# hku-mars/LiDAR_IMU_Init

Hardware: AMD Instinct MI355X
Metric: ICP+ESKF scans/sec @100k pts/scan (higher is better)
Workload: dtype f64; 1 GPU; stream100k: 100000 pts/scan (time-sorted) vs 1000000-pt local map, max_iteration 5, LIO mode (12-col H), static map, voxel-grid leaf 0.05; scans resident in HBM, 8 distinct scans cycled, the state reset to the scan's propagated state every step; map_points=1000000, params=harness/launch/ouster (reference-format yaml + launch), parallelism=points sharded x1, transport=none, rccl_ranks=0

## Files before the change

lidar_imu_init_amd/csrc/lii_capi_register.cpp:

```cpp
#include "lii_context.h"
#include <cstddef>

#include "lii_hostmath.h"

using namespace lii_impl;

namespace {


int next_knn_epoch(lii_handle h) {
  h->knn_epoch = h->knn_epoch >= 0x3FFFFFFE ? 1 : h->knn_epoch + 1;
  return h->knn_epoch;
}
void launch_knn(lii_handle h, const GridView& g, const RegistrationBuffers& rb, const PoseArg* pose, int forced, int epoch,
                hipEvent_t ev_start = nullptr, hipEvent_t ev_stop = nullptr) {
  lii::launch_knn(g, rb, pose, h->d_ctrl, forced, h->d_ctrl->search_pose, h->stream, epoch, ev_start, ev_stop);
}


int iterate(lii_handle h, const lii_state* st, bool search, bool imu_en, double* out91) {
  if (h->n_body <= 0) return fail(h, LII_ERR_STATE, "no down-sampled scan (call lii_downsample / lii_downsample_skip)");
  int rc = commit_map(h);
  if (rc != LII_OK) return rc;
  if (!search && !h->have_search) return fail(h, LII_ERR_STATE, "non-search iteration before any search");
  GridView g = grid_view(h);
  RegistrationBuffers rb = reg_buffers(h);
  const bool prof = h->prof.profiling;
  if (prof) HIPCHK(h, hipEventRecord(h->prof.ev[0], h->stream));
  {
    PoseArg* stage = reinterpret_cast<PoseArg*>(h->h_small + 20000);
    *stage = pose_of(*st);
    HIPCHK(h, hipMemcpyAsync(h->d_pose, stage, sizeof(PoseArg), hipMemcpyHostToDevice, h->stream));
  }
  if (search) h->unfinished_known = false;
  const int epoch = search ? next_knn_epoch(h) : 0;
  if (search) launch_knn(h, g, rb, h->d_pose, 1, epoch);
  if (prof) HIPCHK(h, hipEventRecord(h->prof.ev[3], h->stream));
  launch_fit_reduce(g, rb, h->d_pose, h->d_ctrl, search ? 1 : 0, imu_en ? 1 : 0, h->cfg.plane_threshold,
                    h->cfg.laser_point_cov_inv, h->stream, epoch);
  if (prof) HIPCHK(h, hipEventRecord(h->prof.ev[1], h->stream));
  launch_reduce91(rb, h->d_out91, h->d_ctrl, 1, h->stream, epoch);
  if (prof) HIPCHK(h, hipEventRecord(h->prof.ev[2], h->stream));
  if (search) h->have_search = true;
  if (h->net.comm) {
    ncclResult_t r = ncclAllReduce(h->d_out91, h->d_out91, kNormalEq, ncclDouble, ncclSum, h->net.comm, h->stream);
    if (r != ncclSuccess) return fail(h, LII_ERR_COMM, std::string("ncclAllReduce: ") + ncclGetErrorString(r));
  } else if (h->net.mailbox.dev_slots) {
    launch_mailbox_allreduce(h->d_out91, mailbox_view(h), h->stream);
  }
  HIPCHK(h, hipMemcpyAsync(h->h_small, h->d_out91, sizeof(double) * kNormalEq, hipMemcpyDeviceToHost, h->stream));
  HIPCHK(h, hipStreamSynchronize(h->stream));
  std::memcpy(out91, h->h_small, sizeof(double) * kNormalEq);
  if (h->net.mailbox.dev_slots && out91[kNormalEq - 1] != out91[kNormalEq - 1])
    return fail(h, LII_ERR_COMM, "mailbox exchange timed out (a rank of the job did not reach this pass)");
  if (prof) {
    float a = 0, b = 0;
    HIPCHK(h, hipEventElapsedTime(&a, h->prof.ev[0], h->prof.ev[1]));
    HIPCHK(h, hipEventElapsedTime(&b, h->prof.ev[1], h->prof.ev[2]));
    if (search) {
      float k = 0;
      HIPCHK(h, hipEventElapsedTime(&k, h->prof.ev[0], h->prof.ev[3]));
      h->prof.timings[0] += a; h->prof.timings[5] += 1; h->prof.timings[7] += k;
    } else { h->prof.timings[1] += a; h->prof.timings[6] += 1; }
    h->prof.timings[2] += b;
  }
  return LII_OK;
}

void fill_ctrl(lii_handle h, const lii_state* state, const lii_state* state_prop, const lii_iekf_opts* opts) {
  IekfCtrl* hc = h->h_ctrl;
  std::memcpy(hc->st, state, sizeof(lii_state));
  std::memcpy(hc->prop, state_prop, sizeof(hc->prop));
  hc->max_it = opts->max_iterations;
  hc->imu_en = opts->imu_en;
  hc->it = 0; hc->search_next = 1; hc->stop = 0; hc->rematch_num = 0; hc->converged = 0; hc->searches = 0;
  hc->effect_num = 0; hc->singular = 0;
  h->update_seq = h->update_seq == 0x7FFFFFFF ? 1 : h->update_seq + 1;
  hc->seq = h->update_seq;
  unsigned int plan = 0xFFFFFFFFu;
  if (h->knn_plan && !h->net.comm && opts->max_iterations <= 16) {
    plan = (h->knn_plan_force >= 0 ? ((unsigned int)h->knn_plan_force | 0xFFFF0000u) : h->plan_next) | 0x00010001u;
  }
  hc->plan_mask = plan;
  h->plan_cur = plan;
}

int update_on_device(lii_handle h, lii_state* state, const lii_state* state_prop, const lii_iekf_opts* opts,
                     lii_iekf_report* report) {
  static_assert(sizeof(lii_state) == sizeof(double) * kStateDoubles, "lii_state layout");
  if (h->n_body <= 0) return fail(h, LII_ERR_STATE, "no down-sampled scan (call lii_downsample / lii_downsample_skip)");
  const auto t_map0 = std::chrono::steady_clock::now();
  int rc = commit_map(h);
  if (rc != LII_OK) return rc;
  if (h->diag) h->prof.host_map_us[0] += std::chrono::duration<double, std::micro>(std::chrono::steady_clock::now() - t_map0).count();
  hipStream_t s = h->stream;
  if (!h->map_stream && h->net.n_ranks <= 1) HIPCHK(h, h->map_stream.create(hipStreamNonBlocking));
  if (!h->ctrl_preloaded) {
    if (h->staging_busy) HIPCHK(h, hipStreamSynchronize(s));
    fill_ctrl(h, state, state_prop, opts);
    HIPCHK(h, hipMemcpyAsync(h->d_ctrl, h->h_ctrl, sizeof(IekfCtrl), hipMemcpyHostToDevice, s));
  }
  h->ctrl_preloaded = false;
  h->h_res->singular = 0;
  h->h_res->it = -1;
  if (h->lm.in_job) {
    rc = local_map_enqueue(h, h->d_ctrl->st + 9, nullptr, h->prof.kp_active);
    if (rc != LII_OK) return rc;
  }
  GridView g = grid_view(h);
  RegistrationBuffers rb = reg_buffers(h);
  const PoseArg* pose = reinterpret_cast<const PoseArg*>(h->d_ctrl);
  const bool prof = h->prof.profiling && h->prof.prof_mode != 3;
  if (prof) harvest_knn_events(h);
  const double* ne = h->net.comm ? h->d_out91 + 128 : h->d_out91;
  unsigned int plan = h->plan_cur;
  const unsigned int plan0 = plan;
  auto enqueue_pass = [&](int it) -> int {
    const bool knn = it >= 16 || ((plan >> it) & 1u);
    const int epoch = knn ? next_knn_epoch(h) : 0;
    if (knn) {
      if (h->prof.kp_active) { const int r = kp_mark(h, LII_KP_KNN, it); if (r != LII_OK) return r; }
      if (prof && it < 16) launch_knn(h, g, rb, pose, -1, epoch, h->prof.ev_it[2 * it], h->prof.ev_it[2 * it + 1]);
      else launch_knn(h, g, rb, pose, -1, epoch);
    }
    if (h->prof.kp_active) { const int r = kp_mark(h, LII_KP_FIT, it); if (r != LII_OK) return r; }
    if (knn && h->wide_listed && !h->net.comm && h->net.n_ranks <= 1) launch_complete_listed(g, rb, h->d_ctrl, -1, s, epoch);
    launch_fit_reduce(g, rb, pose, h->d_ctrl, -1, opts->imu_en ? 1 : 0, h->cfg.plane_threshold, h->cfg.laser_point_cov_inv, s, epoch);
    if (h->prof.kp_active) { const int r = kp_mark(h, LII_KP_SOLVE, it); if (r != LII_OK) return r; }
    if (!h->net.comm) {
      launch_reduce_solve(rb, h->d_gran, h->d_ctrl, h->h_res, mailbox_view(h), s, epoch);
      return LII_OK;
    }
    launch_reduce91(rb, h->d_out91, h->d_ctrl, -1, s, epoch);
    ncclResult_t r = ncclAllReduce(h->d_out91, h->d_out91 + 128, kNormalEq, ncclDouble, ncclSum, h->net.comm, s);
    if (r != ncclSuccess) return fail(h, LII_ERR_COMM, std::string("ncclAllReduce: ") + ncclGetErrorString(r));
    launch_iekf_solve(h->d_ctrl, ne, h->h_res, s);
    return LII_OK;
  };
  const auto t_loop0 = std::chrono::steady_clock::now();
  for (int it = 0; it < opts->max_iterations; it++) {
    if (it < 16 && !((plan >> (16 + it)) & 1u)) break;
    rc = enqueue_pass(it);
    if (rc != LII_OK) return rc;
  }
  auto wait_result = [&](bool first) -> int {
    const int parked_word = first ? (h->update_seq | kLoopParked) : h->update_seq;
    if (h->poll_result && !h->net.comm) {
      volatile int* done = &h->h_res->done;
      unsigned int spins = 0;
      while (*done != h->update_seq && *done != parked_word) {
        if ((++spins & 0x3FFF) == 0) {
          const hipError_t q = hipStreamQuery(s);
          if (q == hipSuccess) break;
          if (q != hipErrorNotReady) return fail(h, LII_ERR_HIP, std::string("hipStreamQuery: ") + hipGetErrorString(q));
        }
        __builtin_ia32_pause();
      }
      std::atomic_thread_fence(std::memory_order_acquire);
      if (*done != h->update_seq && *done != parked_word) HIPCHK(h, hipStreamSynchronize(s));
    } else {
      HIPCHK(h, hipStreamSynchronize(s));
    }
    return LII_OK;
  };
  if (h->diag) h->prof.host_loop_enq_us = std::chrono::duration<double, std::micro>(std::chrono::steady_clock::now() - t_loop0).count();
  if (h->prof.kp_active) { rc = kp_mark(h, LII_KP_KINDS); if (rc != LII_OK) return rc; }
  h->map_enqueued_early = false;
  if (h->map_after_update && !h->net.comm && !h->prof.profiling) {
    const auto t_me0 = std::chrono::steady_clock::now();
    h->map_enqueued_early = map_update_early(h) == 1;
    g = grid_view(h);
    if (h->diag) h->prof.host_map_us[1] += std::chrono::duration<double, std::micro>(std::chrono::steady_clock::now() - t_me0).count();
  }
  if (h->pub.on) { rc = publish_enqueue(h, h->d_ctrl, nullptr, true); if (rc != LII_OK) return rc; }
  if (h->pre.want_dev && !h->net.comm && h->net.n_ranks <= 1 && h->prof.prof_mode != 3 && !h->map_async && h->poll_result) {
    lii::GateState* gst = h->pre.state;
    h->pre.seq = (h->pre.seq + 1) & 0x003FFFFFFFFFFFFFull;
    __atomic_store_n(&gst->word, (h->pre.seq << 2) | lii::kGateArmed, __ATOMIC_RELEASE);
    h->pre.scan_dev = h->pre.want_dev; h->pre.n = h->pre.want_n; h->pre.leaf = h->pre.want_leaf; h->pre.late = h->pre.want_late;
    h->pre.fuse = fuse_filter(h, h->pre.leaf);
    DeskewPlan dp = {};
    dp.in = static_cast<const float4*>(h->pre.scan_dev);
    dp.out = h->pre.late ? const_cast<float4*>(dp.in) : h->d_scan;
    dp.n = h->pre.n; dp.sorted = 1; dp.extent = nullptr; dp.bbox_rows = h->d_bbox_rows;
    dp.leaf = h->pre.leaf; dp.vh = h->pre.fuse ? &h->vh : nullptr;
    dp.ctrl_src = h->h_ctrl; dp.ctrl_dst = h->d_ctrl; dp.ctrl_bytes = (sizeof(IekfCtrl) + 15) / 16 * 16;
#ifdef LII_GAP_TRACE
    dp.gap = h->d_gran;
#endif
    lii::DeskewGate gate = {gst, h->pre.d_ring + size_t(h->pre.seq % lii::kGateRing) * lii::kGateLines * 8, h->pre.d_flag, h->pre.seq, h->pre.timeout_ticks, h->pre.late ? 1 : 0};
    launch_deskew_imu_gated(dp, gate, s);
    h->pre.armed = hipGetLastError() == hipSuccess;
    if (!h->pre.armed) __atomic_store_n(&gst->word, (h->pre.seq << 2) | lii::kGateCancel, __ATOMIC_RELEASE);
  }
  h->pre.want_dev = nullptr;
  if (h->wait_hook) {
    void (*hook)(void*) = h->wait_hook;
    h->wait_hook = nullptr;
    h->in_wait_hook = true;
    hook(h->wait_hook_arg);
    h->in_wait_hook = false;
  }
  rc = wait_result(true);
  if (rc != LII_OK) return rc;
  bool parked_once = false;
  for (int round = 0; h->h_res->done == (h->update_seq | kLoopParked); round++) {
    if (round > 2 * opts->max_iterations) return fail(h, LII_ERR_HIP, "device loop parked again and again");
    parked_once = true;
    const int from = h->h_res->parked_it;
    const bool search = h->h_res->parked_search != 0;
    h->plan_parked++;
    prearm_cancel(h);
    h->map_enqueued_early = false;
    g = grid_view(h);
    const int last = std::min(opts->max_iterations, std::max(h->plan_passes_prev, from + 1));
    unsigned int rplan = 0u;
    for (int q = from; q < last && q < 16; q++) rplan |= 1u << (16 + q);
    if (search && from < 16) rplan |= 1u << from;
    plan = rplan;
    h->h_res->done = 0;
    std::atomic_thread_fence(std::memory_order_release);
    launch_loop_resume(h->d_ctrl, rplan, s);
    for (int it = from; it < last; it++) {
      rc = enqueue_pass(it);
      if (rc != LII_OK) return rc;
    }
    if (h->prof.kp_active) { rc = kp_mark(h, LII_KP_KINDS); if (rc != LII_OK) return rc; }
    rc = wait_result(true);
    if (rc != LII_OK) return rc;
  }
  if (h->pub.on && parked_once) {
    if (h->pub.kp_idx >= 0) h->prof.kp_kind[size_t(h->pub.kp_idx)] = LII_KP_KINDS * 64;
    rc = publish_enqueue(h, h->d_ctrl, nullptr, false);
    if (rc != LII_OK) return rc;
  }
  h->unfinished_known = !h->net.comm;
  if (!h->net.comm && h->wide_enabled) {
    const bool wide = h->h_res->unfinished > lii::kFlagCap;
    if (wide == h->wide_prev && wide != h->wide_listed) { h->wide_listed = wide; h->wide_switches++; }
    h->wide_prev = wide;
    if (wide) h->wide_scans++;
  }
  h->staging_busy = false;
  h->scan_buf_idle = !h->pub.on;
  const IekfResult* hr = h->h_res;
  h->have_search = true;
#ifdef LII_SOLVE_TRACE
  {
    static int cnt = 0;
    if (++cnt % 100 == 0) {
      auto row = [&](const long long* t) {
        fprintf(stderr, " loads+sums %lld | A %lld | elimination %lld | solution %lld | state %lld | cov %lld ;", t[1] - t[0], t[2] - t[1], t[4] - t[3], t[8] - t[4],
                t[9] - t[8], t[10] - t[9]);
      };
      fprintf(stderr, "[solve trace, 10 ns ticks] stopping pass:");
      row(hr->ts);
      fprintf(stderr, "  pass 0:");
      row(hr->ts0);
      fprintf(stderr, "\n");
    }
  }
#endif
  if (h->prof.kp_active && h->prof.kp_n > 1 && hr->it > 0) {
    HIPCHK(h, hipEventSynchronize(h->prof.kp_ev[size_t(h->prof.kp_n - 1)]));
    for (int i = 0; i + 1 < h->prof.kp_n; i++) {
      int kind = h->prof.kp_kind[size_t(i)] / 64;
      const int it = h->prof.kp_kind[size_t(i)] % 64;
      if (kind >= LII_KP_KINDS) continue;
      const bool loop_kind = kind == LII_KP_KNN || kind == LII_KP_FIT || kind == LII_KP_SOLVE;
      if (loop_kind && (it >= hr->it || it >= 16)) continue;
      if (kind == LII_KP_KNN && !(hr->search_log[it] & 1)) continue;
      if (kind == LII_KP_FIT && (hr->search_log[it] & 1)) kind = LII_KP_FIT_SEARCH;
      float ms = 0;
      if (hipEventElapsedTime(&ms, h->prof.kp_ev[size_t(i)], h->prof.kp_ev[size_t(i + 1)]) != hipSuccess) continue;
      h->prof.kprof.ms[kind] += ms;
      h->prof.kprof.launches[kind] += 1;
    }
    h->prof.kprof.scans += 1;
  }
  if (hr->part_overflow) {
    h->h_res->part_overflow = 0;
    return fail(h, LII_ERR_CAPACITY, "voxel-partitioned job: this rank's share of the down-sampled cloud exceeds its bound (mean share + 25 % + 2048 points); use lii_comm_set_partition(h, 1)");
  }
  if (hr->singular == 3)
    return fail(h, LII_ERR_COMM, "mailbox exchange timed out (a rank of the job did not reach this pass); re-create the communicator");
  if (hr->singular == 4)
    return fail(h, LII_ERR_COMM, "the sums of a pass did not reach the solver within 2 s (a summing workgroup of the launch was not scheduled: is the device shared?)");
  if (hr->singular) return fail(h, LII_ERR_INVALID, "singular covariance / normal matrix in the device solve");
  if (hr->it < 0) return fail(h, LII_ERR_HIP, "device loop ended without a result");
  std::memcpy(state, hr->st, sizeof(lii_state));
  publish_finish(h);
  h->last_pivoted_passes = 0;
  for (int q = 0; q < 16 && q < hr->it; q++) h->last_pivoted_passes += (hr->search_log[q] >> 1) & 1;
  {
    unsigned int next = 0xFFFFFFFFu;
    for (int q = 0; q < 16 && q < hr->it; q++)
      if (!(hr->search_log[q] & 1)) next &= ~(1u << q);
    for (int q = std::max(hr->it, h->plan_passes_prev); q < 16; q++) next &= ~(1u << (16 + q));
    h->plan_passes_prev = hr->it;
    h->plan_next = next;
  }
  if (report) {
    report->iterations = hr->it;
    report->searches = hr->searches;
    report->effect_num = hr->effect_num;
    report->converged = hr->converged;
    std::memcpy(report->normal_eq, hr->ne, sizeof(double) * kNormalEq);
  }
  if (prof) {
    unsigned int due = 0u;
    for (int it = 0; it < opts->max_iterations && it < 16; it++) {
      if (it >= hr->it || !(hr->search_log[it] & 1) || !((plan0 >> it) & 1u)) continue;
      due |= 1u << it;
    }
    h->prof.ev_it_due = due;
  }
  return LII_OK;
}



int imu_prologue(lii_handle h, const lii_scan_job* job, const ImuFeed* feed, const lii_state* state, bool adopt, const float4* src_dev, int n_next,
                 bool sorted) {
  if (n_next <= 0) return fail(h, LII_ERR_STATE, "lii_scan_register_imu: no scan (lii_scan_upload / lii_frame_select / lii_scan_job::scan_dev)");
  int rc = imu_buffers(h);
  if (rc != LII_OK) return rc;
  if (h->staging_busy) HIPCHK(h, hipStreamSynchronize(h->stream));
  HIPCHK(h, hipEventSynchronize(h->ev_poses));
  h->staging_busy = true;
  fill_ctrl(h, state, state, &job->opts);
  std::memcpy(h->h_poses, feed->imu, sizeof(lii_imu_sample) * size_t(feed->n_imu));
  extent_discard(h);
  h->n_scan = n_next;
  h->n_body = 0;
  h->n_body_pending = false;
  h->have_search = false;
  const float fuse_leaf = job->leaf > 0 ? job->leaf : 0.f;
  h->vh_inserted = fuse_filter(h, fuse_leaf);
  if (h->vh_inserted) h->vh_inserted_leaf = fuse_leaf;
  const float4* in = adopt ? src_dev : h->d_scan.get();
  const unsigned long long* ext = nullptr;
  if (!sorted) {
    unsigned long long* e = h->d_extent + 2 * h->extent_sel;
    launch_time_extent(in, n_next, e, h->d_extent + 2 * (h->extent_sel ^ 1), adopt ? h->d_scan.get() : nullptr, nullptr, nullptr, 0, h->stream);
    h->extent_sel ^= 1;
    ext = e;
    in = h->d_scan;
  }
  ImuPropArgs a = {};
  a.st_in = h->h_ctrl->st;
  a.samples = reinterpret_cast<const double*>(h->h_poses);
  a.n_imu = feed->n_imu;
  static_assert(sizeof(lii_imu_noise) == 8 + 19 * sizeof(double), "lii_imu_noise layout");
  std::memcpy(a.noise, h->imu.noise.cov_gyr, sizeof(a.noise));
  a.pcl_beg_time = feed->pcl_beg_time;
  a.scan = in; a.n_scan = n_next; a.sorted = sorted ? 1 : 0; a.extent = ext;
  a.carry_in = h->imu.d_carry(h->imu.carry_sel);
  a.carry_out = h->imu.d_carry(h->imu.carry_sel ^ 1);
  a.poses = h->d_poses;
  a.n_poses = h->imu.d_n_poses();
  a.st_out = h->d_ctrl->st;
  a.prop_out = h->d_ctrl->prop;
  a.host_out = feed->prop_out ? h->imu.h_out.get() : nullptr;
  a.ctrl_src = reinterpret_cast<const uint4*>(h->h_ctrl);
  a.ctrl_dst = reinterpret_cast<uint4*>(h->d_ctrl);
  static_assert(offsetof(IekfCtrl, solution) % 16 == 0 && offsetof(IekfCtrl, prop) + sizeof(IekfCtrl::prop) == offsetof(IekfCtrl, solution), "IekfCtrl: the two states come first");
  a.ctrl_from = int(offsetof(IekfCtrl, solution) / 16);
  a.ctrl_vec = int((sizeof(IekfCtrl) + 15) / 16);
  launch_imu_propagate(a, h->stream);
  {
    const hipError_t e_prop = hipGetLastError();
    if (e_prop != hipSuccess) { h->vh_inserted = false; return fail(h, LII_ERR_HIP, std::string("IMU propagation launch: ") + hipGetErrorString(e_prop)); }
  }
  h->imu.carry_sel ^= 1;
  if (h->prof.kp_active) { rc = kp_mark(h, LII_KP_DESKEW); if (rc != LII_OK) return rc; }
  DeskewPlan dp = {};
  dp.in = in; dp.out = h->d_scan; dp.n = n_next; dp.sorted = sorted ? 1 : 0; dp.extent = ext; dp.bbox_rows = h->d_bbox_rows;
  dp.leaf = fuse_leaf; dp.vh = h->vh_inserted ? &h->vh : nullptr;
#ifdef LII_GAP_TRACE
  dp.gap = h->d_gran;
#endif
  launch_deskew_imu_dev(dp, h->d_ctrl->st, h->imu.d_n_poses(), h->d_poses, h->stream);
  h->bbox_rows = (n_next + 255) / 256;
  h->ctrl_preloaded = true;
  const hipError_t e_launch = hipGetLastError();
  if (e_launch != hipSuccess) { h->vh_inserted = false; h->ctrl_preloaded = false; return fail(h, LII_ERR_HIP, std::string("de-skew launch behind the IMU propagation: ") + hipGetErrorString(e_launch)); }
  return LII_OK;
}

int cv_prologue(lii_handle h, const lii_scan_job* job, const CvFeed* cv, const lii_state* state, bool adopt, const float4* src_dev, int n_next, bool sorted) {
  if (n_next <= 0) return fail(h, LII_ERR_STATE, "lii_scan_register_cv: no scan (lii_scan_upload / lii_frame_select / lii_scan_job::scan_dev)");
  int rc = LII_OK;
  if (cv->prop_out) { rc = imu_buffers(h); if (rc != LII_OK) return rc; }
  if (h->staging_busy) HIPCHK(h, hipStreamSynchronize(h->stream));
  h->staging_busy = true;
  fill_ctrl(h, state, state, &job->opts);
  extent_discard(h);
  h->n_scan = n_next;
  h->n_body = 0;
  h->n_body_pending = false;
  h->have_search = false;
  const float fuse_leaf = job->leaf > 0 ? job->leaf : 0.f;
  h->vh_inserted = fuse_filter(h, fuse_leaf);
  if (h->vh_inserted) h->vh_inserted_leaf = fuse_leaf;
  const float4* in = adopt ? src_dev : h->d_scan.get();
  const unsigned long long* ext = nullptr;
  if (!sorted) {
    unsigned long long* e = h->d_extent + 2 * h->extent_sel;
    launch_time_extent(in, n_next, e, h->d_extent + 2 * (h->extent_sel ^ 1), adopt ? h->d_scan.get() : nullptr, nullptr, nullptr, 0, h->stream);
    h->extent_sel ^= 1;
    ext = e;
    in = h->d_scan;
  }
  DeskewPlan dp = {};
  dp.in = in; dp.out = h->d_scan; dp.n = n_next; dp.sorted = sorted ? 1 : 0; dp.extent = ext; dp.bbox_rows = h->d_bbox_rows;
  dp.leaf = fuse_leaf; dp.vh = h->vh_inserted ? &h->vh : nullptr;
  dp.ctrl_src = h->h_ctrl; dp.ctrl_dst = h->d_ctrl; dp.ctrl_bytes = (sizeof(IekfCtrl) + 15) / 16 * 16;
#ifdef LII_GAP_TRACE
  dp.gap = h->d_gran;
#endif
  CvFuseH f = {};
  std::memcpy(f.rot, state->rot_end, 72);
  std::memcpy(f.bias_g, state->bias_g, 24);
  std::memcpy(f.vel, state->vel_end, 24);
  f.dt = cv->dt;
  std::memcpy(f.cov_gyr_scale, cv->cov_gyr_scale, 24);
  std::memcpy(f.cov_acc_scale, cv->cov_acc_scale, 24);
  f.st_in = h->h_ctrl->st;
  f.st_out = h->d_ctrl->st;
  f.prop_out = h->d_ctrl->prop;
  f.host_out = cv->prop_out ? h->imu.h_out.get() : nullptr;
  static_assert(offsetof(IekfCtrl, solution) % 16 == 0 && offsetof(IekfCtrl, prop) + sizeof(IekfCtrl::prop) == offsetof(IekfCtrl, solution), "IekfCtrl: the two states come first");
  f.ctrl_from = int(offsetof(IekfCtrl, solution) / 16);
  launch_deskew_cv_prop(dp, f, h->stream);
  h->bbox_rows = (n_next + 255) / 256;
  h->ctrl_preloaded = true;
  const hipError_t e_launch = hipGetLastError();
  if (e_launch != hipSuccess) { h->vh_inserted = false; h->ctrl_preloaded = false; return fail(h, LII_ERR_HIP, std::string("de-skew launch with the CV propagation: ") + hipGetErrorString(e_launch)); }
  return LII_OK;
}

}

int lii_impl::scan_register_job(lii_handle h, const lii_scan_job* job, lii_state* state, const lii_state* state_prop, lii_iekf_report* report,
                                const ImuFeed* feed, const CvFeed* cv) {
  const char* const who = feed ? "lii_scan_register_imu" : (cv ? "lii_scan_register_cv" : "lii_scan_register");
  static_assert(sizeof(lii_scan_job) == 88, "lii_scan_job: the sizes of the earlier ABIs are accepted by number");
  if (!h || !job || (job->struct_size != sizeof(lii_scan_job) && job->struct_size != 72u && job->struct_size != 56u && job->struct_size != 48u) || !state || (!state_prop && !feed && !cv) || job->opts.max_iterations < 1)
    return fail(h, LII_ERR_INVALID, std::string(who) + ": bad arguments");
  const bool sort_first = job->struct_size >= 56u && job->scan_sorted == 2;
  if (sort_first && (h->net.comm || h->net.n_ranks > 1)) return fail(h, LII_ERR_STATE, std::string(who) + ": scan_sorted = 2 is single rank only for now (a communicator is attached)");
  const bool sorted = job->struct_size >= 56u && (job->scan_sorted == 1 || sort_first);
  const bool local_map = h->lm.enabled;
  if (local_map && (h->net.comm || h->net.n_ranks > 1)) return fail(h, LII_ERR_STATE, std::string(who) + ": the local map (lii_local_map_set) is single rank only for now (a communicator is attached)");
  if (local_map && h->host_solve) return fail(h, LII_ERR_STATE, std::string(who) + ": the local map (lii_local_map_set) is not available under LII_TEST=host_solve; call lii_local_map_segment");
  h->scan_buf_idle = false;
  int rc = LII_OK;
  const auto t_entry = std::chrono::steady_clock::now();
  if (h->diag && h->prof.host_us[4] > 0) h->prof.host_us[5] += std::chrono::duration<double, std::micro>(t_entry - h->prof.host_last_return).count();
  const bool from_job = job->scan_dev != nullptr && job->n_scan_dev > 0;
  const void* src_dev = from_job ? job->scan_dev : static_cast<const void*>(h->scan_pending);
  const int src_n = from_job ? job->n_scan_dev : h->scan_pending_n;
  bool adopt = src_dev != nullptr && src_n > 0;
  if (adopt && src_n > h->cfg.max_scan_points) return fail(h, LII_ERR_CAPACITY, std::string(who) + ": n_scan_dev > max_scan_points");
  if (from_job) intensity_detach(h);
  const int n_next = adopt ? src_n : h->n_scan;
  const float leaf_now = job->leaf > 0 ? job->leaf : 0.f;
  const void* const cur_dev = from_job ? job->scan_dev : (adopt ? nullptr : static_cast<const void*>(h->d_scan));
  const int cur_n = from_job ? job->n_scan_dev : h->n_scan;
  bool use_pre = h->pre.armed && sorted && job->undistort == 1 && job->imu_poses && job->n_imu_poses >= 2 && job->n_imu_poses <= lii::kGateMaxPoses &&
                 cur_dev != nullptr && cur_dev == h->pre.scan_dev && cur_n == h->pre.n && h->pre.late == !from_job && leaf_now == h->pre.leaf && !h->host_solve && !h->no_fast_prologue &&
                 h->prof.prof_mode != 3 && !h->staging_busy && fuse_filter(h, leaf_now) == h->pre.fuse;
  if (feed || cv || sort_first || local_map) use_pre = false;
  if (!use_pre) prearm_cancel(h);
  h->pre.want_dev = nullptr;
  if (!feed && !cv && !sort_first && !local_map && job->struct_size >= 72u && job->next_scan_dev && job->next_n_scan > 0 && job->next_n_scan <= h->cfg.max_scan_points && h->pre.enabled &&
      sorted && job->undistort == 1) {
    h->pre.want_dev = job->next_scan_dev; h->pre.want_n = job->next_n_scan; h->pre.want_leaf = leaf_now; h->pre.want_late = false;
  } else if (!feed && !cv && !sort_first && !local_map && h->n_scan_next > 0 && h->d_scan_next && h->pre.enabled && sorted && job->undistort == 1 && !from_job) {
    h->pre.want_dev = h->d_scan_next; h->pre.want_n = h->n_scan_next; h->pre.want_leaf = leaf_now; h->pre.want_late = true;
  }
  h->prof.kp_active = h->prof.prof_mode == 3 && !h->host_solve;
  h->prof.kp_n = 0;
  if (h->prof.kp_active) { rc = kp_mark(h, feed ? LII_KP_PROPAGATE : LII_KP_DESKEW); if (rc != LII_OK) { h->prof.kp_active = false; return rc; } }
  const bool fast = sorted && !h->host_solve && n_next > 0 && !h->no_fast_prologue &&
                    ((job->undistort == 1 && job->imu_poses && job->n_imu_poses >= 2 && job->n_imu_poses <= 64) || job->undistort == 2);
  if (use_pre && !fast) { prearm_cancel(h); use_pre = false; }
  if (job->undistort != 0 && job->undistort != 1 && job->undistort != 2) return fail(h, LII_ERR_INVALID, std::string(who) + ": undistort must be 0, 1 or 2");
  const auto t_first = std::chrono::steady_clock::now();
  if (sort_first && n_next > 0) {
    rc = scan_sort_into(h, adopt ? static_cast<const float4*>(src_dev) : h->d_scan.get(), n_next);
    if (rc != LII_OK) { h->prof.kp_active = false; return rc; }
    extent_discard(h);
    h->n_scan = n_next;
    h->bbox_rows = 0;
    adopt = false;
    src_dev = nullptr;
  }
  if (feed) {
    rc = imu_prologue(h, job, feed, state, adopt, static_cast<const float4*>(src_dev), n_next, sorted);
    if (rc != LII_OK) { h->prof.kp_active = false; return rc; }
  } else if (cv) {
    rc = cv_prologue(h, job, cv, state, adopt, static_cast<const float4*>(src_dev), n_next, sorted);
    if (rc != LII_OK) { h->prof.kp_active = false; return rc; }
  } else if (fast) {
    if (h->staging_busy) HIPCHK(h, hipStreamSynchronize(h->stream));
    h->staging_busy = true;
    fill_ctrl(h, state, state_prop, &job->opts);
    h->ctrl_preloaded = true;
    extent_discard(h);
    h->n_scan = n_next;
    h->n_body = 0;
    h->n_body_pending = false;
    h->have_search = false;
    const float fuse_leaf = job->leaf > 0 ? job->leaf : 0.f;
    h->vh_inserted = fuse_filter(h, fuse_leaf);
    if (h->vh_inserted) h->vh_inserted_leaf = fuse_leaf;
    if (use_pre) {
      h->pre.armed = false;
      if (gate_move(h->pre.state, h->pre.seq, lii::kGateGo)) {
        h->pre.n_used++;
        const int K = job->n_imu_poses;
        const int n_pay = 25 + 22 * K, n_lines = (n_pay + 6) / 7;
        double pay[7 * lii::kGateLines];
        pay[0] = double(K);
        std::memcpy(pay + 1, state->rot_end, 72);
        std::memcpy(pay + 10, state->pos_end, 24);
        std::memcpy(pay + 13, state->offset_R_L_I, 72);
        std::memcpy(pay + 22, state->offset_T_L_I, 24);
        std::memcpy(pay + 25, job->imu_poses, sizeof(lii_pose6d) * size_t(K));
        for (int e = n_pay; e < 7 * n_lines; e++) pay[e] = 0.0;
        volatile double* rec = h->pre.d_ring + size_t(h->pre.seq % lii::kGateRing) * lii::kGateLines * 8;
        double tag;
        const unsigned long long tagw = (h->pre.seq << 2) | lii::kGateGo;
        std::memcpy(&tag, &tagw, 8);
        for (int l = 0; l < n_lines; l++)
          for (int c = 0; c < 7; c++) rec[8 * l + c] = pay[7 * l + c];
        __builtin_ia32_sfence();
        for (int l = 1; l < n_lines; l++) rec[8 * l + 7] = tag;
        __builtin_ia32_sfence();
        {
          const unsigned long long tag0 = tagw | ((unsigned long long)K << 56);
          double t0d;
          std::memcpy(&t0d, &tag0, 8);
          rec[7] = t0d;
        }
        __builtin_ia32_sfence();
      } else {
        use_pre = false;
        h->pre.n_expired++;
      }
    }
    DeskewPlan dp = {};
    dp.in = adopt ? static_cast<const float4*>(src_dev) : h->d_scan;
    dp.out = h->d_scan; dp.n = n_next; dp.sorted = 1; dp.extent = nullptr; dp.bbox_rows = h->d_bbox_rows;
    dp.leaf = fuse_leaf; dp.vh = h->vh_inserted ? &h->vh : nullptr;
// ... 245 lines not shown
```

lidar_imu_init_amd/csrc/lii_iekf.hip:

```cpp
#include <hip/hip_runtime.h>
#include <string.h>
#include <cstring>
#include <math.h>

#include "lii_device.h"
#include "lii_launch.h"

namespace lii {

constexpr int N = 24;
constexpr int H = 12;
constexpr int LDH = 13;

__device__ __forceinline__ double readlane_f64(double v, int lane) {
  union { double d; int i[2]; } u;
  u.d = v;
  u.i[0] = __builtin_amdgcn_readlane(u.i[0], lane);
  u.i[1] = __builtin_amdgcn_readlane(u.i[1], lane);
  return u.d;
}
__device__ __forceinline__ bool gj12_pivoting(double (&col)[H]) {
#pragma unroll
  for (int k = 0; k < H; k++) {
    double mx = 0.0;
    {
      double t[H];
#pragma unroll
      for (int r = 0; r < H; r++) t[r] = r > k ? fabs(col[r]) : 0.0;
#pragma unroll
      for (int w = 1; w < 16; w <<= 1) {
#pragma unroll
        for (int r = 0; r + w < H; r += 2 * w) t[r] = fmax(t[r], t[r + w]);
      }
      mx = t[0];
    }
    const int keep = __builtin_amdgcn_readlane((fabs(col[k]) >= 0.25 * mx) ? 1 : 0, k);
    double m[H];
#pragma unroll
    for (int r = 0; r < H; r++) m[r] = readlane_f64(col[r], k);
    if (!keep) {
      int p = k;
      double best = fabs(m[k]);
#pragma unroll
      for (int r = k + 1; r < H; r++) {
        const double v = fabs(m[r]);
        if (v > best) { best = v; p = r; }
      }
      double colp = col[k], mp = m[k];
#pragma unroll
      for (int r = k + 1; r < H; r++)
        if (r == p) { colp = col[r]; mp = m[r]; col[r] = col[k]; m[r] = m[k]; }
      col[k] = colp;
      m[k] = mp;
    }
    if (!(fabs(m[k]) > 0.0)) return false;
    double inv = __builtin_amdgcn_rcp(m[k]);
    inv = fma(fma(-m[k], inv, 1.0), inv, inv);
    inv = fma(fma(-m[k], inv, 1.0), inv, inv);
    const double rowk = col[k] * inv;
#pragma unroll
    for (int r = 0; r < H; r++)
      if (r != k) col[r] -= m[r] * rowk;
    col[k] = rowk;
  }
  return true;
}

__device__ __forceinline__ float max3_abs(float a, float b, float c) {
  float r;
  asm("v_max3_f32 %0, |%1|, |%2|, |%3|" : "=v"(r) : "v"(a), "v"(b), "v"(c));
  return r;
}
__device__ __forceinline__ float max3_pos(float a, float b, float c) {
  float r;
  asm("v_max3_f32 %0, %1, %2, %3" : "=v"(r) : "v"(a), "v"(b), "v"(c));
  return r;
}
__device__ __forceinline__ float col_absmax_hi(const double (&col)[H], float g) {
  float t[H];
#pragma unroll
  for (int r = 0; r < H; r++) t[r] = __int_as_float(__double2hiint(col[r]));
  const float a = max3_abs(t[0], t[1], t[2]), b = max3_abs(t[3], t[4], t[5]), c = max3_abs(t[6], t[7], t[8]), d = max3_abs(t[9], t[10], t[11]);
  return max3_pos(max3_pos(a, b, c), d, g);
}
__device__ __forceinline__ bool gj12_loop(double (&col)[H]) {
  float g = col_absmax_hi(col, 0.f);
  const unsigned int bound = max(__float_as_uint(g), 0x3FF00000u ) + (8u << 20);
#pragma nounroll
  for (int k = 0; k < H; k++) {
    double m[H];
#pragma unroll
    for (int r = 0; r < H; r++) m[r] = readlane_f64(col[r], k);
    double inv = __builtin_amdgcn_rcp(m[0]);
    inv = fma(fma(-m[0], inv, 1.0), inv, inv);
    inv = fma(fma(-m[0], inv, 1.0), inv, inv);
    const double rowk = col[0] * inv;
#pragma unroll
    for (int r = 1; r < H; r++) col[r - 1] = fma(-m[r], rowk, col[r]);
    col[H - 1] = rowk;
    g = col_absmax_hi(col, g);
  }
  unsigned int top = 0u;
#pragma unroll
  for (int r = 0; r < H; r++) top = max(top, (unsigned int)__double2hiint(col[r]) & 0x7FFFFFFFu);
  return __all(__float_as_uint(g) <= bound && top < 0x7FF00000u);
}
__device__ __forceinline__ bool gj12(double (&col)[H], bool& pivoted) {
  pivoted = false;
  double keep[H];
#pragma unroll
  for (int r = 0; r < H; r++) keep[r] = col[r];
  if (__builtin_expect(gj12_loop(col), 1)) return true;
#pragma unroll
  for (int r = 0; r < H; r++) col[r] = keep[r];
  pivoted = true;
  return gj12_pivoting(col);
}

__device__ void d_m3_mul(const double* A, const double* B, double* C) {
#pragma clang fp contract(off)
  double t[9];
  for (int r = 0; r < 3; r++)
    for (int c = 0; c < 3; c++) t[3 * r + c] = A[3 * r] * B[c] + A[3 * r + 1] * B[3 + c] + A[3 * r + 2] * B[6 + c];
  for (int e = 0; e < 9; e++) C[e] = t[e];
}
__device__ void d_m3t_mul(const double* A, const double* B, double* C) {
#pragma clang fp contract(off)
  double t[9];
  for (int r = 0; r < 3; r++)
    for (int c = 0; c < 3; c++) t[3 * r + c] = A[r] * B[c] + A[3 + r] * B[3 + c] + A[6 + r] * B[6 + c];
  for (int e = 0; e < 9; e++) C[e] = t[e];
}
__device__ void d_so3_exp(double v1, double v2, double v3, double* R) {
#pragma clang fp contract(off)
  double n = sqrt(v1 * v1 + v2 * v2 + v3 * v3);
  for (int e = 0; e < 9; e++) R[e] = (e % 4 == 0) ? 1.0 : 0.0;
  if (n > 0.00001) {
    double ax[3] = {v1 / n, v2 / n, v3 / n};
    double K[9] = {0, -ax[2], ax[1], ax[2], 0, -ax[0], -ax[1], ax[0], 0};
    double cK[9], KK[9];
    double s = sin(n), c1 = 1.0 - cos(n);
    for (int e = 0; e < 9; e++) cK[e] = c1 * K[e];
    d_m3_mul(cK, K, KK);
    for (int e = 0; e < 9; e++) R[e] = (R[e] + s * K[e]) + KK[e];
  }
}
__device__ void d_so3_log(const double* R, double* out) {
#pragma clang fp contract(off)
  double tr = R[0] + R[4] + R[8];
  double theta = (tr > 3.0 - 1e-6) ? 0.0 : acos(0.5 * (tr - 1));
  double K[3] = {R[7] - R[5], R[2] - R[6], R[3] - R[1]};
  double f = (fabs(theta) < 0.001) ? 0.5 : (0.5 * theta / sin(theta));
  out[0] = f * K[0]; out[1] = f * K[1]; out[2] = f * K[2];
}

#ifdef LII_SOLVE_TRACE
#define LII_TS(k) do { if (threadIdx.x == 0) s_ts[k] = wall_clock64(); } while (0)
#else
#define LII_TS(k)
#endif
constexpr int kSolveThreads = 256;
template <class T>
__device__ __forceinline__ void res_store(T* p, T v) { __hip_atomic_store(p, v, __ATOMIC_RELAXED, __HIP_MEMORY_SCOPE_SYSTEM); }
__device__ __forceinline__ void publish_done(IekfResult* res, int seq) {
  asm volatile("s_waitcnt vmcnt(0)" ::: "memory");
  __syncthreads();
  if (threadIdx.x == 0) __hip_atomic_store(&res->done, seq, __ATOMIC_RELAXED, __HIP_MEMORY_SCOPE_SYSTEM);
}

template <class NeSrc>
__device__ __forceinline__ void iekf_solve_body(IekfCtrl* c, IekfResult* res, NeSrc ne_src) {
#ifdef LII_SOLVE_TRACE
  __shared__ long long s_ts[16];
#endif
  LII_TS(0);
  __shared__ double s_cov[N * N];
  __shared__ double G[H * LDH];
  __shared__ double A[H * LDH];
  __shared__ double K1c[N * LDH];
  __shared__ double vec[N], sol[N], s_u[H], s_KH[N * H];
  __shared__ double s_x[N * N];
  __shared__ double s_ne[96], s_st[36], s_prop[36];
  __shared__ int s_int[12];
  __shared__ int s_ok;
  const int tid = threadIdx.x, wave = tid >> 6, lane = tid & 63;
  {
    const int* ci = &c->max_it;
    if (tid < 12) s_int[tid] = ci[tid];
    if (tid >= 160 && tid < 196) { s_st[tid - 160] = c->st[tid - 160]; s_prop[tid - 160] = c->prop[tid - 160]; }
    const double* cov = c->st + 36;
    for (int e = tid; e < N * N; e += kSolveThreads) s_cov[e] = cov[e];
  }
  if (const int why = ne_src(s_ne)) {
    __syncthreads();
    if (threadIdx.x == 0) { c->stop = 1; c->singular = why; res_store(&res->singular, why); res_store(&res->it, 0); }
    publish_done(res, s_int[10]);
    return;
  }
  __syncthreads();
  if (s_int[4]) return;
  LII_TS(1);
  const int max_it = s_int[0], it = s_int[2], search_now = s_int[3], rematch0 = s_int[5], searches0 = s_int[7];
  static const unsigned char kTri[78] = {0, 1, 2, 3, 4, 5, 6, 7, 8, 9, 10, 11, 17, 18, 19, 20, 21, 22, 23, 24, 25, 26, 27, 34, 35, 36, 37, 38, 39, 40, 41, 42, 43, 51, 52, 53, 54, 55, 56, 57, 58, 59, 68, 69, 70, 71, 72, 73, 74, 75, 85, 86, 87, 88, 89, 90, 91, 102, 103, 104, 105, 106, 107, 119, 120, 121, 122, 123, 136, 137, 138, 139, 153, 154, 155, 170, 171, 187};
  if (tid < H * H) {
    const int i = tid / H, j = tid % H;
    double s = (i == j) ? 1.0 : 0.0;
#pragma unroll
    for (int k = 0; k < H; k++) {
      const int a = k < j ? k : j, b = k < j ? j : k;
      s += s_cov[i * N + k] * s_ne[a * H - (a * (a - 1)) / 2 + (b - a)];
    }
    A[i * LDH + j] = s;
  } else if (wave == 3) {
    for (int t = lane; t < 78; t += 64) {
      const int i = kTri[t] >> 4, j = kTri[t] & 15;
      G[i * LDH + j] = s_ne[t];
      G[j * LDH + i] = s_ne[t];
    }
    if (lane >= 32 && lane < 50) {
      const int q = lane - 32, blk = q / 3, i = q % 3;
      const int sto = blk == 0 ? 9 : (blk == 1 ? 21 : (blk == 2 ? 24 : (blk == 3 ? 27 : (blk == 4 ? 30 : 33))));
      const int vo = blk == 0 ? 3 : (blk == 1 ? 9 : (blk == 2 ? 12 : (blk == 3 ? 15 : (blk == 4 ? 18 : 21))));
      vec[vo + i] = s_prop[sto + i] - s_st[sto + i];
    }
  }
  if (tid == 0) s_ok = 1;
  __syncthreads();
  LII_TS(2);
  LII_TS(3);
  if (wave == 0) {
    double col[H];
#pragma unroll
    for (int r = 0; r < H; r++) col[r] = lane < H ? A[r * LDH + lane] : (lane < H + N ? s_cov[r * N + (lane - H)] : 0.0);
    bool pivoted;
    const bool ok = gj12(col, pivoted);
    if (lane == 0) s_ok = ok ? (pivoted ? 2 : 1) : 0;
    if (lane >= H && lane < H + N) {
#pragma unroll
      for (int r = 0; r < H; r++) K1c[(lane - H) * LDH + r] = col[r];
    }
  } else if (wave == 1) {
    if (lane < 2) {
      const int o = lane * 12, so = lane * 6;
      double R[9];
      d_m3t_mul(s_st + o, s_prop + o, R);
      d_so3_log(R, vec + so);
    }
    __builtin_amdgcn_fence(__ATOMIC_SEQ_CST, "wavefront");
    if (lane < H) {
      double s2 = s_ne[78 + lane];
#pragma unroll
      for (int k = 0; k < H; k++) s2 -= G[lane * LDH + k] * vec[k];
      s_u[lane] = s2;
    }
  }
  __syncthreads();
  if (!s_ok) {
    if (tid == 0) { c->stop = 1; c->singular = 1; res_store(&res->singular, 1); }
    publish_done(res, s_int[10]);
    return;
  }
  LII_TS(4);
  if (tid < N) {
    double s2 = vec[tid];
#pragma unroll
    for (int k = 0; k < H; k++) s2 += K1c[tid * LDH + k] * s_u[k];
    sol[tid] = s2;
  }
  __syncthreads();
  LII_TS(8);
  const double rn = sqrt(sol[0] * sol[0] + sol[1] * sol[1] + sol[2] * sol[2]);
  const double tn = sqrt(sol[3] * sol[3] + sol[4] * sol[4] + sol[5] * sol[5]);
  const int converged = (rn * 57.3 < 0.01) && (tn * 100 < 0.015);
  int rematch = rematch0, search = 0;
  if (converged || ((rematch == 0) && (it == (max_it - 2)))) { search = 1; rematch++; }
  const int do_cov = (rematch >= 2 || (it == max_it - 1));
  const unsigned int pm = (unsigned int)s_int[11];
  const bool pass_there = it + 1 >= 16 || ((pm >> (16 + it + 1)) & 1u), knn_there = it + 1 >= 16 || ((pm >> (it + 1)) & 1u);
  const int parked = !do_cov && (!pass_there || (search && !knn_there));
  if (wave == 0) {
    if (lane < 2) {
      double E[9], Rn[9];
      const int o = lane == 0 ? 0 : 12;
      const int so = lane == 0 ? 0 : 6;
      d_so3_exp(sol[so], sol[so + 1], sol[so + 2], E);
      d_m3_mul(s_st + o, E, Rn);
      for (int e = 0; e < 9; e++) c->st[o + e] = Rn[e];
      if (do_cov)
        for (int e = 0; e < 9; e++) res_store(&res->st[o + e], Rn[e]);
    } else if (lane >= 8 && lane < 26) {
      const int q = lane - 8;
      const int blk = q / 3, i = q % 3;
      const int sto = blk == 0 ? 9 : (blk == 1 ? 21 : (blk == 2 ? 24 : (blk == 3 ? 27 : (blk == 4 ? 30 : 33))));
      const int soo = blk == 0 ? 3 : (blk == 1 ? 9 : (blk == 2 ? 12 : (blk == 3 ? 15 : (blk == 4 ? 18 : 21))));
      const double v = s_st[sto + i] + sol[soo + i];
      c->st[sto + i] = v;
      if (do_cov) res_store(&res->st[sto + i], v);
    } else if (lane >= 32 && lane < 32 + N) {
      c->solution[lane - 32] = sol[lane - 32];
    }
    if (lane == 63) {
      c->converged = converged;
      c->rematch_num = rematch;
      c->search_next = search;
      c->effect_num = (int)s_ne[90];
      c->it = it + 1;
      c->searches = searches0 + (search_now ? 1 : 0);
      if (it < 16) c->search_log[it] = search_now | (s_ok == 2 ? 2 : 0);
      if (parked) {
        c->stop = 2;
        res_store(&res->parked_it, it + 1);
        res_store(&res->parked_search, search);
      }
      if (do_cov) {
        c->stop = 1;
        res_store(&res->it, it + 1);
        res_store(&res->searches, searches0 + (search_now ? 1 : 0));
        res_store(&res->effect_num, (int)s_ne[90]);
        res_store(&res->converged, converged);
        res_store(&res->singular, 0);
      }
    }
  } else if (do_cov) {
    const int r0 = 8 * (wave - 1);
    for (int e = lane; e < 8 * H; e += 64) {
      const int r = r0 + e / H, cc = e % H;
      double s2 = 0;
#pragma unroll
      for (int k = 0; k < H; k++) s2 += K1c[r * LDH + k] * G[k * LDH + cc];
      s_KH[r * H + cc] = s2;
    }
    __builtin_amdgcn_fence(__ATOMIC_RELEASE, "wavefront");
    __builtin_amdgcn_wave_barrier();
    __builtin_amdgcn_fence(__ATOMIC_ACQUIRE, "wavefront");
    for (int e = lane; e < 8 * N; e += 64) {
      const int r = r0 + e / N, cc = e % N;
      double s2 = s_cov[r * N + cc];
      for (int k = 0; k < H; k++) s2 -= s_KH[r * H + k] * s_cov[k * N + cc];
      s_x[r * N + cc] = s2;
    }
  }
  LII_TS(9);
  if (do_cov) {
    __syncthreads();
    double* covw = c->st + 36;
    for (int e = tid; e < N * N; e += kSolveThreads) {
      const int r = e / N, cc = e % N;
      const double v = 0.5 * (s_x[e] + s_x[cc * N + r]);
      covw[e] = v;
      res_store(&res->st[36 + e], v);
    }
    if (tid < 91) res_store(&res->ne[tid], s_ne[tid]);
    if (tid >= 96 && tid < 112) {
      const int q = tid - 96;
      res_store(&res->search_log[q], (q < it) ? c->search_log[q] : (q == it ? (search_now | (s_ok == 2 ? 2 : 0)) : 0));
    }
    publish_done(res, s_int[10]);
  } else if (parked) {
    publish_done(res, s_int[10] | kLoopParked);
  }
#ifdef LII_SOLVE_TRACE
  __syncthreads();
  LII_TS(10);
  if (threadIdx.x < 11) { if (it == 0) res->ts0[threadIdx.x] = s_ts[threadIdx.x]; else res->ts[threadIdx.x] = s_ts[threadIdx.x]; }
#endif
}

__device__ __attribute__((noinline, used)) void solve_code_end();
__device__ __forceinline__ int warm_code() {
  const char* pc = reinterpret_cast<const char*>(__builtin_amdgcn_s_getpc() & ~63ull);
  const char* end = reinterpret_cast<const char*>(&solve_code_end);
  int acc = 0;
  if (threadIdx.x < 192) {
#pragma unroll
    for (int u = 0; u < 2; u++) {
      const char* a = pc + (size_t)(threadIdx.x + 192 * u) * 64;
      if (a + 64 <= end) acc ^= *reinterpret_cast<const volatile int*>(a);
    }
  }
  return acc;
}
__device__ __forceinline__ unsigned int pass_tag(int seq, int it) { return ((unsigned int)seq << 6) ^ (unsigned int)(it + 1); }
__global__ __launch_bounds__(kSolveThreads) void k_reduce_solve(const double* __restrict__ partials, int n_blocks, int stride,
                                                                 unsigned long long* __restrict__ gran, IekfCtrl* c, IekfResult* res,
                                                                 MailboxView mb, const int* __restrict__ flag_count) {
  __shared__ double s_w[kSolveThreads / 64];
  const int stop = c->stop, seq = c->seq, it = c->it;
  const int t = blockIdx.x;
  if (t < kNormalEq) {
    const double acc = final_sum_row<kSolveThreads>(partials + (size_t)t * stride, n_blocks, s_w);
    if (stop) return;
    if (threadIdx.x == 0 && !(mb.test_drop_sum && t == 5)) {
      const unsigned int tag = pass_tag(seq, it);
      const unsigned long long b = (unsigned long long)__double_as_longlong(acc);
      __hip_atomic_store(gran + 2 * t, ((unsigned long long)tag << 32) | (b & 0xFFFFFFFFull), __ATOMIC_RELAXED, __HIP_MEMORY_SCOPE_AGENT);
      __hip_atomic_store(gran + 2 * t + 1, ((unsigned long long)tag << 32) | (b >> 32), __ATOMIC_RELAXED, __HIP_MEMORY_SCOPE_AGENT);
    }
    return;
  }
  if (stop) return;
  if (threadIdx.x == kSolveThreads - 1 && flag_count) {
    const int now = max(flag_count[0], flag_count[1]);
    const int before = it == 0 ? 0 : (int)gran[240];
    const int um = max(now, before);
    gran[240] = (unsigned long long)um;
    res_store(&res->unfinished, um);
  }
  const unsigned int tag = pass_tag(seq, it);
  const int warm = warm_code();
  iekf_solve_body(c, res, [&](double* s_ne) {
    __shared__ int s_mb_ok;
    if (threadIdx.x < 64) {
      const int l = threadIdx.x;
      const bool two = l + 64 < kNormalEq;
      const int a = 2 * l, b = two ? 2 * (l + 64) : 2 * l;
      unsigned long long g0, g1, g2, g3;
      unsigned int spins = 0;
      bool arrived = true;
      const long long t0 = wall_clock64();
      for (;;) {
        g0 = __hip_atomic_load(gran + a, __ATOMIC_RELAXED, __HIP_MEMORY_SCOPE_AGENT);
        g1 = __hip_atomic_load(gran + a + 1, __ATOMIC_RELAXED, __HIP_MEMORY_SCOPE_AGENT);
        g2 = __hip_atomic_load(gran + b, __ATOMIC_RELAXED, __HIP_MEMORY_SCOPE_AGENT);
        g3 = __hip_atomic_load(gran + b + 1, __ATOMIC_RELAXED, __HIP_MEMORY_SCOPE_AGENT);
        const bool ok = (unsigned int)(g0 >> 32) == tag && (unsigned int)(g1 >> 32) == tag && (unsigned int)(g2 >> 32) == tag &&
                        (unsigned int)(g3 >> 32) == tag;
        if (__all(ok)) break;
        if ((++spins & 1023u) == 0u && wall_clock64() - t0 > mb.handoff_ticks) { arrived = false; break; }
        __builtin_amdgcn_s_sleep(1);
      }
      double v0 = __longlong_as_double((long long)((g1 << 32) | (g0 & 0xFFFFFFFFull)));
      double v1 = two ? __longlong_as_double((long long)((g3 << 32) | (g2 & 0xFFFFFFFFull))) : 0.0;
      bool ok = true;
      if (arrived && (mb.slots || mb.peers)) ok = mailbox_allreduce(mb, v0, v1);
      s_ne[l] = v0;
      if (two) s_ne[l + 64] = v1;
      if (l == 0) s_mb_ok = !arrived ? 4 : (ok ? 0 : 3);
    }
    if (warm == 0x5EED5EED) s_ne[95] = 0.0;
    __syncthreads();
    return s_mb_ok;
  });
#ifdef LII_GAP_TRACE
  __syncthreads();
  if (threadIdx.x == 0 && c->stop == 1) gran[200] = wall_clock64();
#endif
}

__global__ __launch_bounds__(kSolveThreads) void k_iekf_solve(IekfCtrl* c, const double* __restrict__ ne, IekfResult* res) {
  iekf_solve_body(c, res, [&](double* s_ne) {
    const int tid = threadIdx.x;
    if (tid >= 64 && tid < 64 + 91) s_ne[tid - 64] = ne[tid - 64];
    return 0;
  });
}

__device__ __attribute__((noinline, used)) void solve_code_end() { asm volatile("s_nop 0"); }

__global__ __launch_bounds__(64) void k_mailbox_allreduce(double* out, MailboxView mb) {
  const int l = threadIdx.x;
  double v0 = l < kNormalEq ? out[l] : 0.0, v1 = l + 64 < kNormalEq ? out[l + 64] : 0.0;
  const bool ok = mailbox_allreduce(mb, v0, v1);
  if (l < kNormalEq) out[l] = ok ? v0 : __builtin_nan("");
  if (l + 64 < kNormalEq) out[l + 64] = ok ? v1 : __builtin_nan("");
}

void launch_mailbox_allreduce(double* out91, const MailboxView& mb, hipStream_t s) {
  hipLaunchKernelGGL(k_mailbox_allreduce, dim3(1), dim3(64), 0, s, out91, mb);
}
void launch_reduce_solve(const RegistrationBuffers& rb, unsigned long long* gran, IekfCtrl* c, IekfResult* res, const MailboxView& mb,
                         hipStream_t s, int epoch) {
  const int bound = rb.shard_world > 1 ? (rb.n + rb.shard_world - 1) / rb.shard_world + 1 : rb.n;
  int nb = (bound + kBlock - 1) / kBlock;
  if (nb < 1) nb = 1;
  nb += completion_blocks(epoch);
  hipLaunchKernelGGL(k_reduce_solve, dim3(kNormalEq + 1), dim3(kSolveThreads), 0, s, rb.partials, nb, rb.partial_stride, gran, c, res, mb, rb.flag_count);
}
__global__ void k_loop_resume(IekfCtrl* c, unsigned int plan_mask) {
  c->stop = 0;
  c->plan_mask = plan_mask;
}
void launch_loop_resume(IekfCtrl* c, unsigned int plan_mask, hipStream_t s) { hipLaunchKernelGGL(k_loop_resume, dim3(1), dim3(1), 0, s, c, plan_mask); }
void launch_iekf_solve(IekfCtrl* c, const double* ne, IekfResult* res, hipStream_t s) {
  hipLaunchKernelGGL(k_iekf_solve, dim3(1), dim3(kSolveThreads), 0, s, c, ne, res);
}

}
```

Before: 7505 scans/s.

## Use DPP row-broadcast Gauss-Jordan over two waves and parallelize SO3 boxplus per entry

The 12x12 Gauss-Jordan solve is fully unrolled and replaces per-step readlane with DPP row broadcasts, so each 16-lane row holds its own copy of the H columns. The 24 covariance columns are spread across two waves so the elimination runs in parallel rather than on one wave. The pivoting fallback moves to a separate rare path after the barrier. The rotation boxplus (so3 exp plus a 3x3 multiply) is now computed one matrix entry per lane through LDS with wave barriers, instead of serially on two lanes. The trace printout gains the new timestamps. All of this only shortens a small tail solve kernel, at the cost of an extra branch and extra LDS traffic.

Result: faster. 7787 scans/s, median of 6 (+3.8%).

```diff
diff --git a/lidar_imu_init_amd/csrc/lii_capi_register.cpp b/lidar_imu_init_amd/csrc/lii_capi_register.cpp
--- a/lidar_imu_init_amd/csrc/lii_capi_register.cpp
+++ b/lidar_imu_init_amd/csrc/lii_capi_register.cpp
@@ -250,8 +250,8 @@
     static int cnt = 0;
     if (++cnt % 100 == 0) {
       auto row = [&](const long long* t) {
-        fprintf(stderr, " loads+sums %lld | A %lld | elimination %lld | solution %lld | state %lld | cov %lld ;", t[1] - t[0], t[2] - t[1], t[4] - t[3], t[8] - t[4],
-                t[9] - t[8], t[10] - t[9]);
+        fprintf(stderr, " loads+sums %lld | A %lld | elimination %lld (its own %lld) | solution %lld | state %lld (schedule %lld, rotations %lld, stores %lld) | cov %lld ;",
+                t[1] - t[0], t[2] - t[1], t[4] - t[3], t[5] - t[3], t[8] - t[4], t[9] - t[8], t[6] - t[8], t[7] - t[6], t[9] - t[7], t[10] - t[9]);
       };
       fprintf(stderr, "[solve trace, 10 ns ticks] stopping pass:");
       row(hr->ts);
diff --git a/lidar_imu_init_amd/csrc/lii_iekf.hip b/lidar_imu_init_amd/csrc/lii_iekf.hip
--- a/lidar_imu_init_amd/csrc/lii_iekf.hip
+++ b/lidar_imu_init_amd/csrc/lii_iekf.hip
@@ -83,38 +83,34 @@
   const float a = max3_abs(t[0], t[1], t[2]), b = max3_abs(t[3], t[4], t[5]), c = max3_abs(t[6], t[7], t[8]), d = max3_abs(t[9], t[10], t[11]);
   return max3_pos(max3_pos(a, b, c), d, g);
 }
-__device__ __forceinline__ bool gj12_loop(double (&col)[H]) {
+template <int K>
+__device__ __forceinline__ double rowbcast_f64(double v) {
+  return __builtin_amdgcn_update_dpp(0.0, v, 0x150 + K, 0xF, 0xF, true);
+}
+template <int K>
+__device__ __forceinline__ void gj12_dpp_step(double (&col)[H], float& g) {
+  double m[H];
+#pragma unroll
+  for (int r = 0; r < H; r++) m[r] = rowbcast_f64<K>(col[r]);
+  double inv = __builtin_amdgcn_rcp(m[0]);
+  inv = fma(fma(-m[0], inv, 1.0), inv, inv);
+  inv = fma(fma(-m[0], inv, 1.0), inv, inv);
+  const double rowk = col[0] * inv;
+#pragma unroll
+  for (int r = 1; r < H; r++) col[r - 1] = fma(-m[r], rowk, col[r]);
+  col[H - 1] = rowk;
+  g = col_absmax_hi(col, g);
+}
+__device__ __forceinline__ bool gj12_dpp(double (&col)[H]) {
   float g = col_absmax_hi(col, 0.f);
   const unsigned int bound = max(__float_as_uint(g), 0x3FF00000u ) + (8u << 20);
-#pragma nounroll
-  for (int k = 0; k < H; k++) {
-    double m[H];
-#pragma unroll
-    for (int r = 0; r < H; r++) m[r] = readlane_f64(col[r], k);
-    double inv = __builtin_amdgcn_rcp(m[0]);
-    inv = fma(fma(-m[0], inv, 1.0), inv, inv);
-    inv = fma(fma(-m[0], inv, 1.0), inv, inv);
-    const double rowk = col[0] * inv;
-#pragma unroll
-    for (int r = 1; r < H; r++) col[r - 1] = fma(-m[r], rowk, col[r]);
-    col[H - 1] = rowk;
-    g = col_absmax_hi(col, g);
-  }
+  gj12_dpp_step<0>(col, g); gj12_dpp_step<1>(col, g); gj12_dpp_step<2>(col, g); gj12_dpp_step<3>(col, g);
+  gj12_dpp_step<4>(col, g); gj12_dpp_step<5>(col, g); gj12_dpp_step<6>(col, g); gj12_dpp_step<7>(col, g);
+  gj12_dpp_step<8>(col, g); gj12_dpp_step<9>(col, g); gj12_dpp_step<10>(col, g); gj12_dpp_step<11>(col, g);
   unsigned int top = 0u;
 #pragma unroll
   for (int r = 0; r < H; r++) top = max(top, (unsigned int)__double2hiint(col[r]) & 0x7FFFFFFFu);
   return __all(__float_as_uint(g) <= bound && top < 0x7FF00000u);
-}
-__device__ __forceinline__ bool gj12(double (&col)[H], bool& pivoted) {
-  pivoted = false;
-  double keep[H];
-#pragma unroll
-  for (int r = 0; r < H; r++) keep[r] = col[r];
-  if (__builtin_expect(gj12_loop(col), 1)) return true;
-#pragma unroll
-  for (int r = 0; r < H; r++) col[r] = keep[r];
-  pivoted = true;
-  return gj12_pivoting(col);
 }
 
 __device__ void d_m3_mul(const double* A, const double* B, double* C) {
@@ -152,6 +148,32 @@
   double K[3] = {R[7] - R[5], R[2] - R[6], R[3] - R[1]};
   double f = (fabs(theta) < 0.001) ? 0.5 : (0.5 * theta / sin(theta));
   out[0] = f * K[0]; out[1] = f * K[1]; out[2] = f * K[2];
+}
+
+__device__ __forceinline__ double boxplus_rot_entry(const double* v, const double* R, double* xk, double* xck, double* xe, int e) {
+#pragma clang fp contract(off)
+  const int r = e / 3, cc = e % 3;
+  const double v1 = v[0], v2 = v[1], v3 = v[2];
+  const double n = sqrt(v1 * v1 + v2 * v2 + v3 * v3);
+  const double id = (r == cc) ? 1.0 : 0.0;
+  double E = id;
+  if (n > 0.00001) {
+    const double a = v[r == cc ? 0 : 3 - r - cc] / n;
+    const double k = (r == cc) ? 0.0 : ((cc == (r + 1) % 3) ? -a : a);
+    const double s = sin(n), c1 = 1.0 - cos(n);
+    xk[e] = k;
+    xck[e] = c1 * k;
+    __builtin_amdgcn_fence(__ATOMIC_RELEASE, "wavefront");
+    __builtin_amdgcn_wave_barrier();
+    __builtin_amdgcn_fence(__ATOMIC_ACQUIRE, "wavefront");
+    const double kk = xck[3 * r] * xk[cc] + xck[3 * r + 1] * xk[3 + cc] + xck[3 * r + 2] * xk[6 + cc];
+    E = (id + s * k) + kk;
+  }
+  xe[e] = E;
+  __builtin_amdgcn_fence(__ATOMIC_RELEASE, "wavefront");
+  __builtin_amdgcn_wave_barrier();
+  __builtin_amdgcn_fence(__ATOMIC_ACQUIRE, "wavefront");
+  return R[3 * r] * xe[cc] + R[3 * r + 1] * xe[3 + cc] + R[3 * r + 2] * xe[6 + cc];
 }
 
 #ifdef LII_SOLVE_TRACE
@@ -183,6 +205,7 @@
   __shared__ double s_ne[96], s_st[36], s_prop[36];
   __shared__ int s_int[12];
   __shared__ int s_ok;
+  __shared__ double s_rx[2][3][9];
   const int tid = threadIdx.x, wave = tid >> 6, lane = tid & 63;
   {
     const int* ci = &c->max_it;
@@ -228,18 +251,19 @@
   __syncthreads();
   LII_TS(2);
   LII_TS(3);
-  if (wave == 0) {
+  if (wave < 2) {
+    const int p = lane & 15, j = 16 * wave + 4 * (lane >> 4) + (p - H);
     double col[H];
 #pragma unroll
-    for (int r = 0; r < H; r++) col[r] = lane < H ? A[r * LDH + lane] : (lane < H + N ? s_cov[r * N + (lane - H)] : 0.0);
-    bool pivoted;
-    const bool ok = gj12(col, pivoted);
-    if (lane == 0) s_ok = ok ? (pivoted ? 2 : 1) : 0;
-    if (lane >= H && lane < H + N) {
-#pragma unroll
-      for (int r = 0; r < H; r++) K1c[(lane - H) * LDH + r] = col[r];
-    }
-  } else if (wave == 1) {
+    for (int r = 0; r < H; r++) col[r] = p < H ? A[r * LDH + p] : (j < N ? s_cov[r * N + j] : 0.0);
+    if (!gj12_dpp(col)) {
+      if (lane == 0) s_ok = 3;
+    } else if (p >= H && j < N) {
+#pragma unroll
+      for (int r = 0; r < H; r++) K1c[j * LDH + r] = col[r];
+    }
+    LII_TS(5);
+  } else if (wave == 2) {
     if (lane < 2) {
       const int o = lane * 12, so = lane * 6;
       double R[9];
@@ -255,6 +279,21 @@
     }
   }
   __syncthreads();
+  if (__builtin_expect(s_ok == 3, 0)) {
+    __syncthreads();
+    if (wave == 0) {
+      double col[H];
+#pragma unroll
+      for (int r = 0; r < H; r++) col[r] = lane < H ? A[r * LDH + lane] : (lane < H + N ? s_cov[r * N + (lane - H)] : 0.0);
+      const bool ok = gj12_pivoting(col);
+      if (lane == 0) s_ok = ok ? 2 : 0;
+      if (lane >= H && lane < H + N) {
+#pragma unroll
+        for (int r = 0; r < H; r++) K1c[(lane - H) * LDH + r] = col[r];
+      }
+    }
+    __syncthreads();
+  }
   if (!s_ok) {
     if (tid == 0) { c->stop = 1; c->singular = 1; res_store(&res->singular, 1); }
     publish_done(res, s_int[10]);
@@ -278,17 +317,9 @@
   const unsigned int pm = (unsigned int)s_int[11];
   const bool pass_there = it + 1 >= 16 || ((pm >> (16 + it + 1)) & 1u), knn_there = it + 1 >= 16 || ((pm >> (it + 1)) & 1u);
   const int parked = !do_cov && (!pass_there || (search && !knn_there));
+  LII_TS(6);
   if (wave == 0) {
-    if (lane < 2) {
-      double E[9], Rn[9];
-      const int o = lane == 0 ? 0 : 12;
-      const int so = lane == 0 ? 0 : 6;
-      d_so3_exp(sol[so], sol[so + 1], sol[so + 2], E);
-      d_m3_mul(s_st + o, E, Rn);
-      for (int e = 0; e < 9; e++) c->st[o + e] = Rn[e];
-      if (do_cov)
-        for (int e = 0; e < 9; e++) res_store(&res->st[o + e], Rn[e]);
-    } else if (lane >= 8 && lane < 26) {
+    if (lane >= 8 && lane < 26) {
       const int q = lane - 8;
       const int blk = q / 3, i = q % 3;
       const int sto = blk == 0 ? 9 : (blk == 1 ? 21 : (blk == 2 ? 24 : (blk == 3 ? 27 : (blk == 4 ? 30 : 33))));
@@ -298,6 +329,13 @@
       if (do_cov) res_store(&res->st[sto + i], v);
     } else if (lane >= 32 && lane < 32 + N) {
       c->solution[lane - 32] = sol[lane - 32];
+    }
+    if (lane < 32 && (lane & 15) < 9) {
+      const int rho = lane >> 4, e = lane & 15, o = 12 * rho;
+      const double v = boxplus_rot_entry(sol + 6 * rho, s_st + o, s_rx[rho][0], s_rx[rho][1], s_rx[rho][2], e);
+      LII_TS(7);
+      c->st[o + e] = v;
+      if (do_cov) res_store(&res->st[o + e], v);
     }
     if (lane == 63) {
       c->converged = converged;
```
